# hassony2/handobjectconsist

Measured on AMD Instinct MI355X. Metric: trainmeshwarp iters/sec (render+warp, B=64, 256x256), higher is better.
Workload: dtype f32; 1 GPU; trainmeshwarp.py consist step, per-GPU B=64, 256x256, hand 778v/1552f + object 1002v/2000f (7104 faces after fill-back), ResNet-18 fp32 (MIOpen convolutions, channels-last, + fused HIP BatchNorm/ReLU/residual/max-pool kernels), Adam; global_batch=64, image_size=256, parallelism=dp1

## Files before the change

handobjectconsist_amd/_lib.py:

```python
import ctypes
import os

import torch

_HERE = os.path.dirname(os.path.abspath(__file__))
LIB_PATH = os.environ.get("HOC_LIB_PATH") or os.path.join(_HERE, "libmeshraster_hip.so")
ABI_VERSION = 9
FLAG_REFERENCE_ALGO = 1
FLAG_SPARSE_TILES = 2
FLAG_OUTPUT_ZEROED = 4
FLAG_TILE_PER_WORKGROUP = 8
FLAG_TILE_LIST_CLEARED = 16
FLAG_FORCE_PARTS = 1 << 24
FLAG_ONE_WORKGROUP_PER_IMAGE = 32 << 24
FLAG_PARTS_IN_ONE_LAUNCH = 64 << 24
FLAG_PLAIN_DIVISIONS = 4096 << 8
FLAG_FORCE_GATHER = 32 << 8
FLAG_COUNT_PIXEL_MAP_TERMS = 1024 << 8
CRITERION_L1 = 0
CRITERION_L2 = 1
DTYPE_F32, DTYPE_BF16, DTYPE_U8 = 0, 1, 2
DTYPE_CODES = {torch.float32: DTYPE_F32, torch.bfloat16: DTYPE_BF16, torch.uint8: DTYPE_U8}
IMAGE_DTYPES = (torch.float32, torch.bfloat16)
MASK_DTYPES = (torch.float32, torch.uint8)
# ... 74 lines not shown
    "mr_pair_step_field_offsets": (_I, [_P, _I]),
    "mr_pair_step_sizes": (_I, [_P, _P, _P, _P]),
    "mr_pair_step_forward": (_I, [_P, _P]),
    "mr_pair_step_backward": (_I, [_P, _P]),
    "mr_frames_to_batch_workspace_bytes": (_L, [_I, _I, _I]),
    "mr_frames_to_batch": (_I, [_P] * 3 + [_F] * 6 + [_P, _L, _P, _P] + [_I] * 6 + [_P]),
    "mr_frames_to_batch_typed": (_I, [_P] * 3 + [_F] * 6 + [_P, _L, _P, _P] + [_I] * 6 + [_P, _I, _I]),
    "mr_frames_color_augment_workspace_bytes": (_L, [_I, _I, _I]),
    "mr_frames_color_augment": (_I, [_P] * 7 + [_L, _I, _I, _I, _P]),
    "mr_jpeg_info": (_I, [_P, _L, _P]),
    "mr_jpeg_packed_bytes": (_L, [_I] * 5),
    "mr_jpeg_entropy_decode": (_I, [_P, _L, _P, _L]),
    "mr_jpeg_reconstruct_workspace_bytes": (_L, [_I] * 6),
    "mr_jpeg_reconstruct": (_I, [_P] + [_I] * 6 + [_P, _P, _L, _P]),
    "mr_png_packed_bytes": (_L, [_I] * 3),
    "mr_png_unfilter_workspace_bytes": (_L, [_I] * 4),
    "mr_png_unfilter": (_I, [_P] + [_I] * 4 + [_P, _P, _P]),
    "mr_bn_act_forward": (_I, [_P] * 6 + [_F, _I, _I, _I, _P, _I, _I, _I, _P]),
    "mr_bn_act_backward_workspace_bytes": (_L, [_I, _I]),
    "mr_bn_act_backward": (_I, [_P] * 8 + [_F, _I, _I, _I] + [_P] * 5 + [_L, _I, _I, _I, _P]),
    "mr_bn_add_bn_act_forward": (_I, [_P] * 6 + [_F] + [_P] * 4 + [_F, _I, _P, _I, _I, _I, _P]),
    "mr_bn_add_bn_act_backward_workspace_bytes": (_L, [_I, _I]),
    "mr_bn_add_bn_act_backward": (_I, [_P] * 8 + [_F] + [_P] * 4 + [_F, _I] + [_P] * 7 + [_L, _I, _I, _I, _P]),
    "mr_stem_pool_forward": (_I, [_P] * 5 + [_F, _I, _I, _P, _P, _I, _I, _I, _I, _P]),
    "mr_stem_pool_records_bytes": (_L, [_I, _I, _I, _I]),
    "mr_stem_pool_backward_workspace_bytes": (_L, [_I, _I, _I, _I]),
    "mr_stem_pool_backward": (_I, [_P] * 8 + [_F, _I, _I] + [_P] * 4 + [_L, _I, _I, _I, _I, _P]),
    "mr_stem_pool_param_grads": (_I, [_P] * 7 + [_F, _I] + [_P] * 3 + [_L, _I, _I, _I, _I, _P]),
    "mr_stem_conv_wrw_tiling": (_I, [_P] * 3),
    "mr_stem_conv_wrw_workspace_bytes": (_L, [_I, _I, _I, _I]),
    "mr_stem_conv_wrw": (_I, [_P] * 7 + [_F, _P, _P, _I, _P, _L] + [_I] * 8 + [_P]),
}

_lib = None


def load():
    global _lib
    if _lib is not None:
        return _lib
    if not os.path.exists(LIB_PATH):
        raise RuntimeError(
            f"{LIB_PATH} is missing: the HIP extension has not been built. Run "
            "`python -c 'import __graft_entry__ as g; g.build()'` (or `python handobjectconsist_amd/build.py`). "
            "There is no CPU / PyTorch fallback for the render + warp path."
        )
# ... 92 lines not shown
```

handobjectconsist_amd/csrc/frozen_bn.hip:

```cpp
#include "bn_device.hpp"

namespace mr {

struct BnParams {
    const void* x;
    const void* residual;
    BnAffine bn;
    int relu;
    int N, C, HW, split;
    void* y;
    const void* grad_y;
    const void* grad_y2;
    void* grad_x;
    void* grad_residual;
    float* partial;
};

template <bool BACKWARD>
__device__ __forceinline__ void bn_act_element(float x, bool has_res, float res, float grad, bool relu, float mean, float a,
                                               float b, float& out, float& gres, float& sum_g, float& sum_gd) {
    const float d = x - mean;
    float z = d * a + b;
    if (has_res) z = z + res;
    if (!BACKWARD) {
// ... 56 lines not shown
constexpr int BN_NHWC_BLOCKS = 2048;

template <typename T, bool BACKWARD>
__global__ __launch_bounds__(256) void bn_act_nhwc_kernel(BnParams p) {
    const NhwcLane l = nhwc_lane(p.bn, p.C);
    const int64_t pixels = (int64_t)p.N * p.HW;
    const bool relu = p.relu != 0, has_res = p.residual != nullptr;
    float s[2][4] = {};
    for (int64_t px = l.first(); px < pixels; px += l.stride()) {
        const int64_t o = px * p.C + l.c0;
        float xv[4], rv[4] = {}, gv[4] = {}, out[4], gres[4];
        load4<T>(p.x, o, xv);
        if (has_res) load4<T>(p.residual, o, rv);
        if (BACKWARD) load4_grad<T>(p.grad_y, p.grad_y2, o, gv);
#pragma unroll
        for (int i = 0; i < 4; i++)
            bn_act_element<BACKWARD>(xv[i], has_res, rv[i], gv[i], relu, l.mean[i], l.a[i], l.b[i], out[i], gres[i], s[0][i], s[1][i]);
        store4<T>(BACKWARD ? p.grad_x : p.y, o, out);
        if (BACKWARD && p.grad_residual) store4<T>(p.grad_residual, o, gres);
    }
    if (BACKWARD && p.partial) nhwc_block_sums<2>(l, s, p.partial, p.C);
}

struct BnAddParams {
    const void* x;
    const void* xd;
    BnAffine bn, bn_d;
    int N, C, HW;
    void* y;
    const void* grad_y;
    const void* grad_y2;
    void* grad_x;
    void* grad_xd;
    float* partial;
};

template <typename T, bool BACKWARD>
__global__ __launch_bounds__(256) void bn_add_bn_act_nhwc_kernel(BnAddParams p) {
    const NhwcLane l = nhwc_lane(p.bn, p.C), ld = nhwc_lane(p.bn_d, p.C);
    const int64_t pixels = (int64_t)p.N * p.HW;
    float s[3][4] = {};
    for (int64_t px = l.first(); px < pixels; px += l.stride()) {
        const int64_t o = px * p.C + l.c0;
        float xv[4], dv[4], gv[4], out[4], outd[4];
        load4<T>(p.x, o, xv);
        load4<T>(p.xd, o, dv);
// ... 99 lines not shown
    if (channels == 0) return MR_OK;
    if (!weight || !bias || !running_mean || !running_var) return MR_ERR_BADARG;
    const bool want_params = grad_weight || grad_bias;
    if (batch_size == 0 || plane == 0) return zero_param_grads({grad_weight, grad_bias}, channels, (hipStream_t)stream);
    if (!grad_y || !x || !grad_x) return MR_ERR_BADARG;
    if (grad_residual && !residual) return MR_ERR_BADARG;
    if (want_params && (!workspace || workspace_bytes < mr_bn_act_backward_workspace_bytes(batch_size, channels)))
        return MR_ERR_BADARG;
    BnParams p = bn_fill(x, residual, weight, bias, running_mean, running_var, eps, relu, batch_size, channels, plane);
    p.grad_y = grad_y; p.grad_y2 = grad_y2; p.grad_x = grad_x; p.grad_residual = grad_residual;
    p.partial = want_params ? static_cast<float*>(workspace) : nullptr;
    if (!bn_sizes_ok(p)) return MR_ERR_BADARG;
    const bool all_aligned = aligned4(x, act_dtype) && aligned4(grad_y, act_dtype) && aligned4(grad_y2, act_dtype) &&
                             aligned4(grad_x, act_dtype) && aligned4(residual, act_dtype) && aligned4(grad_residual, act_dtype);
    if (channels_last && !all_aligned) return MR_ERR_BADARG;
    const int64_t slots = bn_act_slots(batch_size, channels, channels_last, (int64_t)batch_size * plane);
    bn_launch<true>(p, act_dtype, channels_last, plane % 4 == 0 && all_aligned, (int)slots, (hipStream_t)stream);
    MR_CHECK_LAUNCH();
    if (!want_params) return MR_OK;
    return launch_bn_finish<2>(p.partial, slots, channels, BnFinishOut{running_var, eps, grad_weight, grad_bias}, (hipStream_t)stream);
}

namespace mr {
static BnAddParams bn_add_fill(const void* x, const void* xd, const BnAffine& bn, const BnAffine& bn_d, int N, int C, int plane) {
    BnAddParams p{};
    p.x = x; p.xd = xd; p.bn = bn; p.bn_d = bn_d; p.N = N; p.C = C; p.HW = plane;
    return p;
}
template <bool BACKWARD>
static void bn_add_launch(const BnAddParams& p, int act_dtype, int blocks, hipStream_t s) {
    dispatch_act(act_dtype, [&](auto tag) {
        using T = typename decltype(tag)::type;
        hipLaunchKernelGGL((bn_add_bn_act_nhwc_kernel<T, BACKWARD>), dim3((unsigned)blocks), dim3(256), 0, s, p);
    });
}
}

extern "C" int mr_bn_add_bn_act_forward(const void* x, const void* xd, const float* weight, const float* bias,
                                        const float* running_mean, const float* running_var, float eps,
                                        const float* weight_d, const float* bias_d, const float* running_mean_d,
                                        const float* running_var_d, float eps_d, int act_dtype, void* y, int batch_size,
                                        int channels, int plane, mr_stream_t stream) {
    using namespace mr;
    if (batch_size < 0 || channels < 0 || plane < 0 || (act_dtype != 0 && act_dtype != 1)) return MR_ERR_BADARG;
    if (channels > 0 && !nhwc_channels_ok(channels)) return MR_ERR_BADARG;
    if (batch_size == 0 || channels == 0 || plane == 0) return MR_OK;
// ... 53 lines not shown
```

handobjectconsist_amd/csrc/mano_lbs.hip:

```cpp
#include "mr_common.hpp"

namespace mr {

constexpr int MN_V = 778, MN_J = 16, MN_NV3 = MN_V * 3, MN_KP = 146;
constexpr int MN_TIPS = 5, MN_JT = MN_J + MN_TIPS;
constexpr int MN_SPLITK = 32;

typedef float f32x16 __attribute__((ext_vector_type(16)));

struct ManoConst {
    const float* comps;
    const float* mean;
    const float* js;
    const float* jt;
    const float* blend;
    const float* templ;
    const float* weights;
    const int* parents;
    const int* tips;
    const int* reorder;
    int ncomps, center;
};

struct ManoFull {
    const float* trans;
    int ntrans;
    float* tflag;
    float out_scale;
    const float* post_trans;
    const float* post_rot;
    const float* post_trans2;
};
constexpr int MN_POSE_PCA = 0, MN_POSE_AXISANG = 1;

__device__ __forceinline__ void rigid_mul(const float* A, const float* B, float* C) {
#pragma unroll
    for (int r = 0; r < 3; r++) {
#pragma unroll
        for (int c = 0; c < 4; c++) {
            float v = fmaf(A[4 * r + 2], B[8 + c], fmaf(A[4 * r + 1], B[4 + c], A[4 * r] * B[c]));
            if (c == 3) v += A[4 * r + 3];
            C[4 * r + c] = v;
        }
    }
}

template <int FORM, bool FULL>
__global__ void __launch_bounds__(64) mano_pre_kernel(ManoConst mc, ManoFull mf, const float* __restrict__ pose,
                                                      const float* __restrict__ betas, float* __restrict__ coeff,
                                                      float* __restrict__ G, float* __restrict__ G2,
                                                      float* __restrict__ rots, float* __restrict__ joints,
                                                      float* __restrict__ full_pose_out, float* __restrict__ jtr_out,
                                                      int B) {
    __shared__ float s_pose[48], s_R[MN_J * 9], s_J[48], s_G[MN_J * 12];
    const int b = blockIdx.x, lane = threadIdx.x;
    const int np = FORM == MN_POSE_AXISANG ? 48 : 3 + mc.ncomps;
    if (lane < 3) s_pose[lane] = pose[b * np + lane];
    if (lane < 45) {
        if constexpr (FORM == MN_POSE_AXISANG) {
            s_pose[3 + lane] = mc.mean[lane] + pose[b * np + 3 + lane];
        } else {
            float acc = 0.0f;
            for (int c = 0; c < mc.ncomps; c++) acc = fmaf(pose[b * np + 3 + c], mc.comps[c * 45 + lane], acc);
            s_pose[3 + lane] = mc.mean[lane] + acc;
        }
    }
    if constexpr (FULL) {
        unsigned bits = 0u;
        for (int i = lane; i < mf.ntrans; i += 64) bits |= __float_as_uint(mf.trans[i]) & 0x7fffffffu;
        const bool in_force = __ballot(bits != 0u) != 0ull;
        if (lane == 0) mf.tflag[b] = in_force ? 1.0f : 0.0f;
    }
    if (lane < 48) {
        float acc = 0.0f;
#pragma unroll
        for (int k = 0; k < 10; k++) acc = fmaf(betas[b * 10 + k], mc.js[lane * 10 + k], acc);
        s_J[lane] = acc + mc.jt[lane];
    }
    __syncthreads();
    if (lane < 48) {
        full_pose_out[b * 48 + lane] = s_pose[lane];
        joints[b * 48 + lane] = s_J[lane];
    }
    if (lane < MN_J) {
        float R[9];
        rodrigues(&s_pose[3 * lane], R, nullptr);
#pragma unroll
        for (int k = 0; k < 9; k++) {
            s_R[lane * 9 + k] = R[k];
            rots[(b * MN_J + lane) * 9 + k] = R[k];
            if (lane > 0) coeff[b * MN_KP + 10 + (lane - 1) * 9 + k] = R[k] - ((k == 0 || k == 4 || k == 8) ? 1.0f : 0.0f);
        }
    }
    if (lane < 10) coeff[b * MN_KP + lane] = betas[b * 10 + lane];
    if (lane == 10) coeff[b * MN_KP + MN_KP - 1] = 0.0f;
    __syncthreads();
    if (lane == 0) {
        for (int j = 0; j < MN_J; j++) {
            const int pa = mc.parents[j];
            float rel[12];
#pragma unroll
            for (int r = 0; r < 3; r++) {
#pragma unroll
                for (int c = 0; c < 3; c++) rel[4 * r + c] = s_R[j * 9 + 3 * r + c];
                rel[4 * r + 3] = pa < 0 ? s_J[3 * j + r] : s_J[3 * j + r] - s_J[3 * pa + r];
            }
            if (pa < 0) {
#pragma unroll
                for (int k = 0; k < 12; k++) s_G[j * 12 + k] = rel[k];
            } else {
                rigid_mul(&s_G[pa * 12], rel, &s_G[j * 12]);
            }
        }
    }
    __syncthreads();
    for (int k = lane; k < MN_J * 12; k += 64) {
        const int j = k / 12, e = k % 12, r = e / 4, c = e % 4;
        float v = s_G[k];
        G[b * MN_J * 12 + k] = v;
        if (c == 3)
            v = v - fmaf(s_G[j * 12 + 4 * r + 2], s_J[3 * j + 2],
                         fmaf(s_G[j * 12 + 4 * r + 1], s_J[3 * j + 1], s_G[j * 12 + 4 * r] * s_J[3 * j]));
        G2[b * MN_J * 12 + k] = v;
    }
    if constexpr (!FULL) {
        if (lane < MN_JT * 3) {
            const int k = lane / 3, r = lane % 3, src = mc.reorder[k];
            if (src < MN_J) {
                const float ctr = mc.center >= 0 ? s_G[mc.center * 12 + 4 * r + 3] : 0.0f;
                jtr_out[(b * MN_JT + k) * 3 + r] = (s_G[src * 12 + 4 * r + 3] - ctr) * 1000.0f;
            }
        }
    }
}

__global__ void __launch_bounds__(64) mano_blend_kernel(const float* __restrict__ coeff, const float* __restrict__ blend,
                                                        const float* __restrict__ templ, float* __restrict__ v_posed,
                                                        int B) {
    const int lane = threadIdx.x;
    const int n0 = blockIdx.x * 32, m0 = blockIdx.y * 32;
    const int i = lane & 31, kh = lane >> 5;
    const int row = min(m0 + i, B - 1), col = min(n0 + i, MN_NV3 - 1);
    f32x16 acc = {0, 0, 0, 0, 0, 0, 0, 0, 0, 0, 0, 0, 0, 0, 0, 0};
#pragma unroll 4
    for (int k = 0; k < MN_KP; k += 2) {
        const float a = coeff[row * MN_KP + k + kh];
        const float bb = blend[(k + kh) * MN_NV3 + col];
        acc = __builtin_amdgcn_mfma_f32_32x32x2f32(a, bb, acc, 0, 0, 0);
    }
    const int n = n0 + i;
// ... 221 lines not shown
        acc = __builtin_amdgcn_mfma_f32_32x32x2f32(a, bb, acc, 0, 0, 0);
    }
    const int n = n0 + i;
#pragma unroll
    for (int r = 0; r < 16; r++) {
        const int m = m0 + (r & 3) + 8 * (r >> 2) + 4 * kh;
        if (m < Mpad && n < 160) partial[((int64_t)s * Mpad + m) * 160 + n] = acc[r];
    }
}

template <int FORM, bool FULL>
__global__ void __launch_bounds__(64) mano_pre_bwd_kernel(ManoConst mc, ManoFull mf, float* __restrict__ grad_trans,
                                                          const float* __restrict__ full_pose,
                                                          const float* __restrict__ rots,
                                                          const float* __restrict__ joints, const float* __restrict__ G,
                                                          const float* __restrict__ part,
                                                          const float* __restrict__ partial,
                                                          const float* __restrict__ grad_jtr,
                                                          float* __restrict__ grad_pose, float* __restrict__ grad_betas,
                                                          int B, int Mpad) {
    __shared__ double s_gG2[MN_J * 12], s_gc[3], s_gcoef[MN_KP], s_gG[MN_J * 12], s_gRd[MN_J * 9], s_gJ[48], s_gt[MN_J][3];
    __shared__ float s_gR[MN_J * 9], s_gp[48];
    __shared__ float s_G[MN_J * 12], s_R[MN_J * 9], s_J[48];
    const int b = blockIdx.x, lane = threadIdx.x;
    const int np = FORM == MN_POSE_AXISANG ? 48 : 3 + mc.ncomps;
    for (int k = lane; k < MN_J * 12; k += 64) {
        double acc = 0.0;
        for (int c = 0; c < MN_CHUNKS; c++) acc += (double)part[((int64_t)b * MN_CHUNKS + c) * MN_PART + k];
        s_gG2[k] = acc;
        s_G[k] = G[b * MN_J * 12 + k];
    }
    if (lane < 3) {
        double acc = 0.0;
        for (int c = 0; c < MN_CHUNKS; c++) acc += (double)part[((int64_t)b * MN_CHUNKS + c) * MN_PART + MN_J * 12 + lane];
        s_gc[lane] = acc;
    }
    for (int k = lane; k < MN_KP; k += 64) {
        double acc = 0.0;
        for (int s = 0; s < MN_SPLITK; s++) acc += (double)partial[((int64_t)s * Mpad + b) * 160 + k];
        s_gcoef[k] = acc;
    }
    for (int k = lane; k < MN_J * 9; k += 64) s_R[k] = rots[b * MN_J * 9 + k];
    if (lane < 48) { s_J[lane] = joints[b * 48 + lane]; s_gJ[lane] = 0.0; }
    __syncthreads();
    if (lane == 0) {
        double (*gt)[3] = s_gt;
        for (int j = 0; j < MN_J; j++) gt[j][0] = gt[j][1] = gt[j][2] = 0.0;
        double gc[3] = {s_gc[0], s_gc[1], s_gc[2]};
        if (grad_jtr)
            for (int k = 0; k < MN_JT; k++) {
                const int src = mc.reorder[k];
                for (int r = 0; r < 3; r++) {
                    const double g = (double)grad_jtr[(b * MN_JT + k) * 3 + r] * 1000.0;
                    if (src < MN_J) { gt[src][r] += g; gc[r] -= g; }
                }
            }
        if constexpr (FULL) {
            const bool in_force = mf.tflag[b] != 0.0f;
            if (grad_trans)
                for (int r = 0; r < 3; r++) grad_trans[b * 3 + r] = in_force ? (float)(0.0 - gc[r]) : 0.0f;
            if (mc.center >= 0 && mc.center < MN_J && !in_force)
                for (int r = 0; r < 3; r++) gt[mc.center][r] += gc[r];
        } else {
            if (mc.center >= 0)
                for (int r = 0; r < 3; r++) gt[mc.center][r] += gc[r];
        }
        for (int j = 0; j < MN_J; j++) {
            for (int r = 0; r < 3; r++) {
                const double gt2 = s_gG2[j * 12 + 4 * r + 3];
                for (int c = 0; c < 3; c++) {
                    s_gG[j * 12 + 4 * r + c] = s_gG2[j * 12 + 4 * r + c] - gt2 * (double)s_J[3 * j + c];
                    s_gJ[3 * j + c] -= (double)s_G[j * 12 + 4 * r + c] * gt2;
                }
                s_gG[j * 12 + 4 * r + 3] = gt2 + gt[j][r];
            }
        }
        for (int j = MN_J - 1; j >= 0; j--) {
            const int pa = mc.parents[j];
            if (pa < 0) {
                for (int r = 0; r < 3; r++) {
                    for (int c = 0; c < 3; c++) s_gRd[j * 9 + 3 * r + c] = s_gG[j * 12 + 4 * r + c];
                    s_gJ[3 * j + r] += s_gG[j * 12 + 4 * r + 3];
                }
                continue;
            }
            double rel[12];
            for (int r = 0; r < 3; r++) {
                for (int c = 0; c < 3; c++) rel[4 * r + c] = (double)s_R[j * 9 + 3 * r + c];
                rel[4 * r + 3] = (double)s_J[3 * j + r] - (double)s_J[3 * pa + r];
            }
            for (int r = 0; r < 3; r++)
                for (int c = 0; c < 4; c++) {
                    double acc = 0.0;
                    for (int k = 0; k < 3; k++) acc += (double)s_G[pa * 12 + 4 * k + r] * s_gG[j * 12 + 4 * k + c];
                    if (c < 3) s_gRd[j * 9 + 3 * r + c] = acc;
                    else { s_gJ[3 * j + r] += acc; s_gJ[3 * pa + r] -= acc; }
                }
            for (int r = 0; r < 3; r++) {
                for (int c = 0; c < 3; c++) {
                    double acc = 0.0;
                    for (int k = 0; k < 4; k++) acc += s_gG[j * 12 + 4 * r + k] * rel[4 * c + k];
                    s_gG[pa * 12 + 4 * r + c] += acc;
                }
                s_gG[pa * 12 + 4 * r + 3] += s_gG[j * 12 + 4 * r + 3];
            }
        }
    }
    __syncthreads();
    for (int k = lane; k < MN_J * 9; k += 64) s_gR[k] = (float)(k >= 9 ? s_gRd[k] + s_gcoef[10 + (k - 9)] : s_gRd[k]);
    __syncthreads();
    if (lane < MN_J) {
        float gr[3];
        rodrigues_bwd(&full_pose[b * 48 + 3 * lane], &s_gR[lane * 9], gr);
#pragma unroll
        for (int k = 0; k < 3; k++) s_gp[3 * lane + k] = gr[k];
    }
    __syncthreads();
    if (lane < 3) grad_pose[b * np + lane] = s_gp[lane];
    if constexpr (FORM == MN_POSE_AXISANG) {
        if (lane < 45) grad_pose[b * np + 3 + lane] = s_gp[3 + lane];
    } else if (lane < mc.ncomps) {
        float acc = 0.0f;
        for (int l = 0; l < 45; l++) acc = fmaf(mc.comps[lane * 45 + l], s_gp[3 + l], acc);
        grad_pose[b * np + 3 + lane] = acc;
    }
    if (lane < 10) {
        double acc = s_gcoef[lane];
        for (int l = 0; l < 48; l++) acc += (double)mc.js[l * 10 + lane] * s_gJ[l];
        grad_betas[b * 10 + lane] = (float)acc;
    }
}

}

using namespace mr;

static ManoConst mano_const(const float* comps, const float* mean, const float* js, const float* jt, const float* blend,
                            const float* templ, const float* weights, const int32_t* parents, const int32_t* tips,
                            const int32_t* reorder, int ncomps, int center) {
    return ManoConst{comps, mean, js, jt, blend, templ, weights, (const int*)parents, (const int*)tips, (const int*)reorder,
                     ncomps, center};
}

struct ManoWork {
    float *coeff, *G, *G2, *rots, *joints, *full_pose, *v_posed, *grad_vp, *part, *partial;
    float* tflag;
    int Mpad;
    int64_t floats, full_floats;
};
static ManoWork mano_work(float* w, int64_t B) {
// ... 167 lines not shown
```

handobjectconsist_amd/models/synthnet.py:

```python
import os

import numpy as np
import torch
import torch.nn.functional as F
from torch import nn

from handobjectconsist_amd import _lib
from handobjectconsist_amd.nn import frozen_bn
from handobjectconsist_amd.utils import project as camproject
from handobjectconsist_amd.utils import synth


USE_HIP_BN = os.environ.get("HOC_HIP_BN", "1") == "1"


USE_CHANNELS_LAST = os.environ.get("HOC_CHANNELS_LAST", "1") == "1"


USE_STEM_WRW = True


def _fused_bn(bn, x):
    if not (USE_HIP_BN and not bn.training and x.is_cuda):
        return False
    out_dtype = torch.get_autocast_dtype("cuda") if torch.is_autocast_enabled("cuda") else x.dtype
    return out_dtype in (torch.float32, torch.bfloat16)


class BasicBlock(nn.Module):
    expansion = 1

    def __init__(self, inplanes, planes, stride=1, downsample=None):
        super().__init__()
        self.conv1 = nn.Conv2d(inplanes, planes, 3, stride, 1, bias=False)
        self.bn1 = nn.BatchNorm2d(planes)
        self.relu = nn.ReLU(inplace=True)
        self.conv2 = nn.Conv2d(planes, planes, 3, 1, 1, bias=False)
        self.bn2 = nn.BatchNorm2d(planes)
        self.downsample = downsample

    def forward_fused(self, x, x_identity, dup=False):
        if self.downsample is not None:
            xd = self.downsample[0](x_identity)
            out = frozen_bn.bn_act(self.conv1(x), self.bn1)
            return frozen_bn.bn_add_bn_act(self.conv2(out), self.bn2, xd, self.downsample[1], dup=dup)
        out = frozen_bn.bn_act(self.conv1(x), self.bn1)
        return frozen_bn.bn_act(self.conv2(out), self.bn2, residual=x_identity, dup=dup)

    def forward(self, x):
        if _fused_bn(self.bn1, x):
            return self.forward_fused(x, x)
        residual = x if self.downsample is None else self.downsample(x)
        out = self.relu(self.bn1(self.conv1(x)))
        out = self.bn2(self.conv2(out))
        return self.relu(out + residual)


class ResNet18Features(nn.Module):

    def __init__(self):
        super().__init__()
        self.inplanes = 64
        self.conv1 = nn.Conv2d(3, 64, kernel_size=7, stride=2, padding=3, bias=False)
        self.bn1 = nn.BatchNorm2d(64)
        self.relu = nn.ReLU(inplace=True)
        self.maxpool = nn.MaxPool2d(kernel_size=3, stride=2, padding=1)
        self.layer1 = self._make_layer(64, 2)
        self.layer2 = self._make_layer(128, 2, stride=2)
        self.layer3 = self._make_layer(256, 2, stride=2)
        self.layer4 = self._make_layer(512, 2, stride=2)
# ... 4 lines not shown
    def _make_layer(self, planes, blocks, stride=1):
        downsample = None
        if stride != 1 or self.inplanes != planes:
            downsample = nn.Sequential(nn.Conv2d(self.inplanes, planes, 1, stride, bias=False),
                                       nn.BatchNorm2d(planes))
        layers = [BasicBlock(self.inplanes, planes, stride, downsample)]
        self.inplanes = planes
        layers += [BasicBlock(planes, planes) for _ in range(1, blocks)]
        return nn.Sequential(*layers)

    def forward(self, x):
        if USE_CHANNELS_LAST and x.is_cuda:
            if not self.conv1.weight.is_contiguous(memory_format=torch.channels_last):
                self.to(memory_format=torch.channels_last)
            x = x.contiguous(memory_format=torch.channels_last)
        if _fused_bn(self.bn1, x):
            blocks = [b for layer in (self.layer1, self.layer2, self.layer3, self.layer4) for b in layer]
            if USE_STEM_WRW and frozen_bn.conv_stem_applies(x, self.conv1, self.bn1):
                pair = frozen_bn.conv_stem_pool(x, self.conv1, self.bn1, dup=True)
            else:
                pair = frozen_bn.stem_pool(self.conv1(x), self.bn1, dup=True)
            for block in blocks[:-1]:
                pair = block.forward_fused(pair[0], pair[1], dup=True)
            x = blocks[-1].forward_fused(pair[0], pair[1])
        else:
            x = self.maxpool(self.relu(self.bn1(self.conv1(x))))
            x = self.layer4(self.layer3(self.layer2(self.layer1(x))))
        return x.mean(3).mean(2)


class AbsoluteBranch(nn.Module):

    def __init__(self, base_neurons=(512, 256), out_dim=3):
        super().__init__()
        layers = []
        for i, o in zip(base_neurons[:-1], base_neurons[1:]):
            layers += [nn.Linear(i, o), nn.ReLU()]
        self.decoder = nn.Sequential(*layers)
        self.final_layer = nn.Linear(base_neurons[-1], out_dim)

    def forward(self, inp):
        return self.final_layer(self.decoder(inp))


def batch_rodrigues(rvec):
    angle = torch.norm(rvec + 1e-8, p=2, dim=1, keepdim=True)
    axis = rvec / angle
    half = angle * 0.5
    q = torch.cat([torch.cos(half), torch.sin(half) * axis], 1)
    q = q / q.norm(p=2, dim=1, keepdim=True)
# ... 439 lines not shown
```

handobjectconsist_amd/nn/frozen_bn.py:

```python
import torch
import torch.nn.functional as F

from handobjectconsist_amd import _lib


_ACT_DTYPES = {torch.float32: 0, torch.bfloat16: 1}


def _nhwc_channels_ok(C):
    return 4 <= C <= 1024 and 1024 % C == 0


def _layout(x):
    if (x.dim() == 4 and _nhwc_channels_ok(x.shape[1]) and not x.is_contiguous()
            and x.is_contiguous(memory_format=torch.channels_last)):
        return x, 1
    return x.contiguous(), 0


def _aligned(t, cl):
    if t is not None and cl and t.data_ptr() % (4 * t.element_size()):
        return t.clone(memory_format=torch.preserve_format)
    return t

# ... 51 lines not shown
        xc, rc, w, b, m, v = ctx.saved_tensors
        eps, relu, N, C, plane, cl = ctx.cfg
        need_x, need_r, need_w, need_b = ctx.needs_input_grad[:4]
        g, g2 = _incoming(grad_y, grad_y2, xc.dtype, cl)
        if g is None:
            return (None,) * 9
        dev = xc.device
        grad_x = torch.empty_like(xc)
        grad_r = torch.empty_like(xc) if (rc is not None and need_r) else None
        grad_w = torch.empty_like(w) if need_w else None
        grad_b = torch.empty_like(b) if need_b else None
        work, wbytes = _workspace("mr_bn_act_backward_workspace_bytes", (N, C), dev, need_w or need_b)
        _lib.call("mr_bn_act_backward", _lib.ptr(g), _lib.ptr(g2), _lib.ptr(xc), _lib.ptr(rc), _lib.ptr(w), _lib.ptr(b), _lib.ptr(m),
                  _lib.ptr(v), eps, int(relu), _ACT_DTYPES[xc.dtype], cl, _lib.ptr(grad_x), _lib.ptr(grad_r), _lib.ptr(grad_w),
                  _lib.ptr(grad_b),
                  _lib.ptr(work), wbytes, N, C, plane, _lib.stream_ptr(dev))
        return (grad_x if need_x else None), grad_r, grad_w, grad_b, None, None, None, None, None


def bn_act(x, bn, residual=None, relu=True, dup=False):
    if bn.training or not bn.track_running_stats:
        raise RuntimeError("bn_act needs frozen BatchNorm statistics (module.eval())")
    return _BnActFunction.apply(x, residual, bn.weight, bn.bias, bn.running_mean, bn.running_var, bn.eps, relu, dup)


class _BnAddBnActFunction(torch.autograd.Function):

    @staticmethod
    def forward(ctx, x, xd, weight, bias, running_mean, running_var, eps, weight_d, bias_d, running_mean_d,
                running_var_d, eps_d, dup):
        ctx.set_materialize_grads(False)
        _lib.check_cuda(x, xd, weight, bias, running_mean, running_var, weight_d, bias_d, running_mean_d, running_var_d)
        xc, xdc = _aligned(x, 1), _aligned(xd, 1)
        N, C = xc.shape[:2]
        plane = xc[0, 0].numel() if N and C else 0
        chan = _channel_arrays(C, weight, bias, running_mean, running_var, weight_d, bias_d, running_mean_d, running_var_d)
        y = torch.empty_like(xc)
        _lib.call("mr_bn_add_bn_act_forward", _lib.ptr(xc), _lib.ptr(xdc), *[_lib.ptr(t) for t in chan[:4]], float(eps),
                  *[_lib.ptr(t) for t in chan[4:]], float(eps_d), _ACT_DTYPES[xc.dtype], _lib.ptr(y), N, C, plane,
                  _lib.stream_ptr(xc.device))
        ctx.save_for_backward(xc, xdc, *chan)
        ctx.cfg = (float(eps), float(eps_d), N, C, plane)
        return (y, y.view_as(y)) if dup else y

    @staticmethod
    def backward(ctx, grad_y, grad_y2=None):
# ... 152 lines not shown
```

include/meshraster_hip.h:

```cpp
#ifndef MESHRASTER_HIP_H
#define MESHRASTER_HIP_H

#include <stdint.h>

#ifdef __cplusplus
extern "C" {
#endif

#define MR_OK 0
#define MR_ERR_BADARG (-1)
#define MR_ERR_NOTIMPL (-2)

#define MR_FLAG_REFERENCE_ALGO 1
#define MR_FLAG_SPARSE_TILES 2
#define MR_FLAG_OUTPUT_ZEROED 4
#define MR_FLAG_TILE_PER_WORKGROUP 8
#define MR_FLAG_TILE_LIST_CLEARED 16
#define MR_FLAG_FORCE_PARTS (1 << 24)
#define MR_FLAG_ONE_WORKGROUP_PER_IMAGE (32 << 24)
#define MR_FLAG_PARTS_IN_ONE_LAUNCH (64 << 24)
#define MR_FLAG_PLAIN_DIVISIONS (4096 << 8)
#define MR_FLAG_FORCE_GATHER (32 << 8)
#define MR_FLAG_COUNT_PIXEL_MAP_TERMS (1024 << 8)

// ... 481 lines not shown
MR_API int mr_bn_act_backward(const void* grad_y, const void* grad_y2, const void* x, const void* residual,
                              const float* weight, const float* bias, const float* running_mean,
                              const float* running_var, float eps, int relu, int act_dtype,
                              int channels_last, void* grad_x, void* grad_residual, float* grad_weight,
                              float* grad_bias,
                              void* workspace, int64_t workspace_bytes, int batch_size, int channels,
                              int plane, mr_stream_t stream);

MR_API int mr_bn_add_bn_act_forward(const void* x, const void* xd, const float* weight, const float* bias,
                                    const float* running_mean, const float* running_var, float eps,
                                    const float* weight_d, const float* bias_d, const float* running_mean_d,
                                    const float* running_var_d, float eps_d, int act_dtype, void* y,
                                    int batch_size, int channels, int plane, mr_stream_t stream);
MR_API int64_t mr_bn_add_bn_act_backward_workspace_bytes(int batch_size, int channels);
MR_API int mr_bn_add_bn_act_backward(const void* grad_y, const void* grad_y2, const void* x, const void* xd,
                                     const float* weight, const float* bias, const float* running_mean,
                                     const float* running_var, float eps, const float* weight_d,
                                     const float* bias_d, const float* running_mean_d, const float* running_var_d,
                                     float eps_d, int act_dtype, void* grad_x, void* grad_xd, float* grad_weight,
                                     float* grad_bias, float* grad_weight_d, float* grad_bias_d, void* workspace,
                                     int64_t workspace_bytes, int batch_size, int channels, int plane,
                                     mr_stream_t stream);

MR_API int mr_stem_pool_forward(const void* x, const float* weight, const float* bias,
                                const float* running_mean, const float* running_var, float eps,
                                int act_dtype, int channels_last, void* y, unsigned char* argmax,
                                int batch_size, int channels, int height, int width, mr_stream_t stream);
MR_API int64_t mr_stem_pool_records_bytes(int batch_size, int channels, int height, int width);
MR_API int64_t mr_stem_pool_backward_workspace_bytes(int batch_size, int channels, int height, int width);
MR_API int mr_stem_pool_backward(const void* grad_y, const void* grad_y2, const void* x,
                                 const unsigned char* argmax,
                                 const float* weight, const float* bias, const float* running_mean,
                                 const float* running_var, float eps, int act_dtype, int channels_last,
                                 void* grad_x, float* grad_weight, float* grad_bias, void* workspace,
                                 int64_t workspace_bytes, int batch_size, int channels, int height,
                                 int width, mr_stream_t stream);

MR_API int mr_stem_pool_param_grads(const void* grad_y, const void* grad_y2, const unsigned char* records,
                                    const float* weight, const float* bias, const float* running_mean,
                                    const float* running_var, float eps, int act_dtype, float* grad_weight,
                                    float* grad_bias, void* workspace, int64_t workspace_bytes, int batch_size,
                                    int channels, int height, int width, mr_stream_t stream);

MR_API int mr_stem_conv_wrw_tiling(int* tile_height, int* tile_width, int* workgroups);
MR_API int64_t mr_stem_conv_wrw_workspace_bytes(int batch_size, int channels, int in_height, int in_width);
MR_API int mr_stem_conv_wrw(const float* grad_y, const float* grad_y2, const unsigned char* records,
// ... 11 lines not shown
```

Before: 38.58 iters/s (one optimiser step = 1 data batch + 1 consist batch of B per GPU; roofline.stock_trunk_it_s = the same step with the trunk's BatchNorm/ReLU/max-pool on the stock nn modules).

## Fuse final BN/ReLU/residual with global average pool and parallelise MANO kinematic chain

Adds a fused kernel that applies the last block's frozen BatchNorm, residual add and ReLU and directly reduces to pooled features. Its backward broadcasts the pooled gradient inside the BN backward, which removes the full-size activation write and the separate mean reductions at the trunk exit. It also rewrites the MANO forward and backward kinematic-chain passes from a single serial lane to level-by-level parallel work over chain depth. That adds extra shared memory and syncthreads in exchange. The layer4 output is tiny (8x8), so the gain from the fusion is likely small.

```diff
diff --git a/handobjectconsist_amd/_lib.py b/handobjectconsist_amd/_lib.py
--- a/handobjectconsist_amd/_lib.py
+++ b/handobjectconsist_amd/_lib.py
@@ -120,6 +120,8 @@
     "mr_bn_add_bn_act_forward": (_I, [_P] * 6 + [_F] + [_P] * 4 + [_F, _I, _P, _I, _I, _I, _P]),
     "mr_bn_add_bn_act_backward_workspace_bytes": (_L, [_I, _I]),
     "mr_bn_add_bn_act_backward": (_I, [_P] * 8 + [_F] + [_P] * 4 + [_F, _I] + [_P] * 7 + [_L, _I, _I, _I, _P]),
+    "mr_bn_act_pool_forward": (_I, [_P] * 6 + [_F, _P, _I, _I, _I, _I, _P]),
+    "mr_bn_act_pool_backward": (_I, [_P] * 7 + [_F] + [_P] * 5 + [_L, _I, _I, _I, _I, _P]),
     "mr_stem_pool_forward": (_I, [_P] * 5 + [_F, _I, _I, _P, _P, _I, _I, _I, _I, _P]),
     "mr_stem_pool_records_bytes": (_L, [_I, _I, _I, _I]),
     "mr_stem_pool_backward_workspace_bytes": (_L, [_I, _I, _I, _I]),
diff --git a/handobjectconsist_amd/csrc/frozen_bn.hip b/handobjectconsist_amd/csrc/frozen_bn.hip
--- a/handobjectconsist_amd/csrc/frozen_bn.hip
+++ b/handobjectconsist_amd/csrc/frozen_bn.hip
@@ -102,6 +102,89 @@
     if (BACKWARD && p.partial) nhwc_block_sums<2>(l, s, p.partial, p.C);
 }
 
+struct BnPoolParams {
+    const float* x;
+    const float* residual;
+    BnAffine bn;
+    int N, C, H, W;
+    float inv_h, inv_w;
+    float* features;
+    const float* grad_features;
+    float* grad_x;
+    float* grad_residual;
+    float* partial;
+};
+
+template <int S>
+__device__ __forceinline__ void pool_tree(float (&t)[S][4]) {
+#pragma unroll
+    for (int step = 1; step < S; step *= 2)
+#pragma unroll
+        for (int j = 0; j < S; j += 2 * step)
+#pragma unroll
+            for (int i = 0; i < 4; i++) t[j][i] = t[j][i] + t[j + step][i];
+}
+
+template <int S>
+__global__ __launch_bounds__(256) void bn_act_pool_forward_kernel(BnPoolParams p) {
+    const int groups = p.C >> 2;
+    const int64_t t = (int64_t)blockIdx.x * 256 + threadIdx.x;
+    if (t >= (int64_t)p.N * groups) return;
+    const int n = (int)(t / groups), c0 = 4 * (int)(t % groups);
+    float mean[4], a[4], b[4];
+#pragma unroll
+    for (int i = 0; i < 4; i++) channel_consts(p.bn, c0 + i, mean[i], a[i], b[i]);
+    const bool has_res = p.residual != nullptr;
+    float rows[S][4];
+#pragma unroll
+    for (int h = 0; h < S; h++) {
+        float row[S][4];
+#pragma unroll
+        for (int w = 0; w < S; w++) {
+            const int64_t o = (((int64_t)n * S + h) * S + w) * p.C + c0;
+            float xv[4], rv[4] = {};
+            load4<float>(p.x, o, xv);
+            if (has_res) load4<float>(p.residual, o, rv);
+#pragma unroll
+            for (int i = 0; i < 4; i++) {
+                float gres, s0 = 0.0f, s1 = 0.0f;
+                bn_act_element<false>(xv[i], has_res, rv[i], 0.0f, true, mean[i], a[i], b[i], row[w][i], gres, s0, s1);
+            }
+        }
+        pool_tree<S>(row);
+#pragma unroll
+        for (int i = 0; i < 4; i++) rows[h][i] = row[0][i] * p.inv_w;
+    }
+    pool_tree<S>(rows);
+    float f[4];
+#pragma unroll
+    for (int i = 0; i < 4; i++) f[i] = rows[0][i] * p.inv_h;
+    store4<float>(p.features, (int64_t)n * p.C + c0, f);
+}
+
+__global__ __launch_bounds__(256) void bn_act_pool_backward_kernel(BnPoolParams p) {
+    const NhwcLane l = nhwc_lane(p.bn, p.C);
+    const int HW = p.H * p.W;
+    const int64_t pixels = (int64_t)p.N * HW;
+    const bool has_res = p.residual != nullptr;
+    float s[2][4] = {};
+    for (int64_t px = l.first(); px < pixels; px += l.stride()) {
+        const int64_t o = px * p.C + l.c0;
+        float xv[4], rv[4] = {}, gv[4], out[4], gres[4];
+        load4<float>(p.x, o, xv);
+        if (has_res) load4<float>(p.residual, o, rv);
+        load4<float>(p.grad_features, (px / HW) * p.C + l.c0, gv);
+#pragma unroll
+        for (int i = 0; i < 4; i++) {
+            const float g = (gv[i] * p.inv_h) * p.inv_w;
+            bn_act_element<true>(xv[i], has_res, rv[i], g, true, l.mean[i], l.a[i], l.b[i], out[i], gres[i], s[0][i], s[1][i]);
+        }
+        store4<float>(p.grad_x, o, out);
+        if (p.grad_residual) store4<float>(p.grad_residual, o, gres);
+    }
+    if (p.partial) nhwc_block_sums<2>(l, s, p.partial, p.C);
+}
+
 struct BnAddParams {
     const void* x;
     const void* xd;
@@ -247,6 +330,77 @@
 }
 
 namespace mr {
+static int bn_pool_check(int N, int C, int H, int W, std::initializer_list<const void*> ptrs) {
+    if (N < 0 || C < 0 || H < 0 || W < 0) return MR_ERR_BADARG;
+    if (C > 0 && !nhwc_channels_ok(C)) return MR_ERR_BADARG;
+    if ((int64_t)H * W > 0x7fffffff || (int64_t)N * C > 0x7fffffff) return MR_ERR_BADARG;
+    for (const void* q : ptrs)
+        if (!aligned4(q, 0)) return MR_ERR_BADARG;
+    return MR_OK;
+}
+static BnPoolParams bn_pool_fill(const void* x, const void* residual, const float* weight, const float* bias, const float* mean,
+                                 const float* var, float eps, int N, int C, int H, int W) {
+    BnPoolParams p{};
+    p.x = static_cast<const float*>(x); p.residual = static_cast<const float*>(residual);
+    p.bn = BnAffine{weight, bias, mean, var, eps};
+    p.N = N; p.C = C; p.H = H; p.W = W;
+    p.inv_h = 1.0f / (float)H; p.inv_w = 1.0f / (float)W;
+    return p;
+}
+}
+
+extern "C" int mr_bn_act_pool_forward(const void* x, const void* residual, const float* weight, const float* bias,
+                                      const float* running_mean, const float* running_var, float eps, float* features,
+                                      int batch_size, int channels, int height, int width, mr_stream_t stream) {
+    using namespace mr;
+    const int rc = bn_pool_check(batch_size, channels, height, width, {x, residual, features});
+    if (rc != MR_OK) return rc;
+    if (batch_size == 0 || channels == 0) return MR_OK;
+    if (height == 0 || width == 0) return MR_ERR_BADARG;
+    if (!x || !weight || !bias || !running_mean || !running_var || !features) return MR_ERR_BADARG;
+    if (height != width || (height != 1 && height != 2 && height != 4 && height != 8)) return MR_ERR_NOTIMPL;
+    BnPoolParams p = bn_pool_fill(x, residual, weight, bias, running_mean, running_var, eps, batch_size, channels, height, width);
+    p.features = features;
+    const dim3 grid((unsigned)(((int64_t)batch_size * (channels / 4) + 255) / 256));
+    switch (height) {
+        case 1: hipLaunchKernelGGL(bn_act_pool_forward_kernel<1>, grid, dim3(256), 0, (hipStream_t)stream, p); break;
+        case 2: hipLaunchKernelGGL(bn_act_pool_forward_kernel<2>, grid, dim3(256), 0, (hipStream_t)stream, p); break;
+        case 4: hipLaunchKernelGGL(bn_act_pool_forward_kernel<4>, grid, dim3(256), 0, (hipStream_t)stream, p); break;
+        default: hipLaunchKernelGGL(bn_act_pool_forward_kernel<8>, grid, dim3(256), 0, (hipStream_t)stream, p); break;
+    }
+    MR_CHECK_LAUNCH();
+    return MR_OK;
+}
+
+extern "C" int mr_bn_act_pool_backward(const float* grad_features, const void* x, const void* residual, const float* weight,
+                                       const float* bias, const float* running_mean, const float* running_var, float eps,
+                                       void* grad_x, void* grad_residual, float* grad_weight, float* grad_bias,
+                                       void* workspace, int64_t workspace_bytes, int batch_size, int channels, int height,
+                                       int width, mr_stream_t stream) {
+    using namespace mr;
+    const int rc = bn_pool_check(batch_size, channels, height, width, {grad_features, x, residual, grad_x, grad_residual});
+    if (rc != MR_OK) return rc;
+    if (channels == 0) return MR_OK;
+    if (!weight || !bias || !running_mean || !running_var) return MR_ERR_BADARG;
+    const bool want_params = grad_weight || grad_bias;
+    if (batch_size == 0) return zero_param_grads({grad_weight, grad_bias}, channels, (hipStream_t)stream);
+    if (height == 0 || width == 0) return MR_ERR_BADARG;
+    if (!grad_features || !x || !grad_x) return MR_ERR_BADARG;
+    if (grad_residual && !residual) return MR_ERR_BADARG;
+    if (want_params && (!workspace || workspace_bytes < mr_bn_act_backward_workspace_bytes(batch_size, channels)))
+        return MR_ERR_BADARG;
+    BnPoolParams p = bn_pool_fill(x, residual, weight, bias, running_mean, running_var, eps, batch_size, channels, height, width);
+    p.grad_features = grad_features;
+    p.grad_x = static_cast<float*>(grad_x); p.grad_residual = static_cast<float*>(grad_residual);
+    p.partial = want_params ? static_cast<float*>(workspace) : nullptr;
+    const int64_t slots = bn_act_slots(batch_size, channels, 1, (int64_t)batch_size * height * width);
+    hipLaunchKernelGGL(bn_act_pool_backward_kernel, dim3((unsigned)slots), dim3(256), 0, (hipStream_t)stream, p);
+    MR_CHECK_LAUNCH();
+    if (!want_params) return MR_OK;
+    return launch_bn_finish<2>(p.partial, slots, channels, BnFinishOut{running_var, eps, grad_weight, grad_bias}, (hipStream_t)stream);
+}
+
+namespace mr {
 static BnAddParams bn_add_fill(const void* x, const void* xd, const BnAffine& bn, const BnAffine& bn_d, int N, int C, int plane) {
     BnAddParams p{};
     p.x = x; p.xd = xd; p.bn = bn; p.bn_d = bn_d; p.N = N; p.C = C; p.HW = plane;
diff --git a/handobjectconsist_amd/csrc/mano_lbs.hip b/handobjectconsist_amd/csrc/mano_lbs.hip
--- a/handobjectconsist_amd/csrc/mano_lbs.hip
+++ b/handobjectconsist_amd/csrc/mano_lbs.hip
@@ -45,6 +45,20 @@
     }
 }
 
+__device__ __forceinline__ int chain_depths(int parent, int* s_par, int* s_depth, int lane) {
+    if (lane < MN_J) s_par[lane] = parent;
+    __syncthreads();
+    if (lane < MN_J) {
+        int d = 0;
+        for (int p = s_par[lane]; p >= 0 && p < MN_J && d < MN_J; p = s_par[p]) d++;
+        s_depth[lane] = d;
+    }
+    __syncthreads();
+    int maxd = 0;
+    for (int j = 0; j < MN_J; j++) maxd = max(maxd, s_depth[j]);
+    return maxd;
+}
+
 template <int FORM, bool FULL>
 __global__ void __launch_bounds__(64) mano_pre_kernel(ManoConst mc, ManoFull mf, const float* __restrict__ pose,
                                                       const float* __restrict__ betas, float* __restrict__ coeff,
@@ -53,8 +67,11 @@
                                                       float* __restrict__ full_pose_out, float* __restrict__ jtr_out,
                                                       int B) {
     __shared__ float s_pose[48], s_R[MN_J * 9], s_J[48], s_G[MN_J * 12];
+    __shared__ int s_par[MN_J], s_depth[MN_J];
     const int b = blockIdx.x, lane = threadIdx.x;
     const int np = FORM == MN_POSE_AXISANG ? 48 : 3 + mc.ncomps;
+    const int parent = lane < MN_J ? mc.parents[lane] : -1;
+    const int src = !FULL && lane < MN_JT * 3 ? mc.reorder[lane / 3] : MN_J;
     if (lane < 3) s_pose[lane] = pose[b * np + lane];
     if (lane < 45) {
         if constexpr (FORM == MN_POSE_AXISANG) {
@@ -94,26 +111,26 @@
     }
     if (lane < 10) coeff[b * MN_KP + lane] = betas[b * 10 + lane];
     if (lane == 10) coeff[b * MN_KP + MN_KP - 1] = 0.0f;
-    __syncthreads();
-    if (lane == 0) {
-        for (int j = 0; j < MN_J; j++) {
-            const int pa = mc.parents[j];
-            float rel[12];
-#pragma unroll
-            for (int r = 0; r < 3; r++) {
-#pragma unroll
-                for (int c = 0; c < 3; c++) rel[4 * r + c] = s_R[j * 9 + 3 * r + c];
-                rel[4 * r + 3] = pa < 0 ? s_J[3 * j + r] : s_J[3 * j + r] - s_J[3 * pa + r];
+    const int maxd = chain_depths(parent, s_par, s_depth, lane);
+    for (int d = 0; d <= maxd; d++) {
+        for (int k = lane; k < MN_J * 12; k += 64) {
+            const int j = k / 12, r = (k % 12) / 4, c = k % 4;
+            if (s_depth[j] != d) continue;
+            const int pa = s_par[j];
+            float rel[3];
+#pragma unroll
+            for (int i = 0; i < 3; i++)
+                rel[i] = c < 3 ? s_R[j * 9 + 3 * i + c] : (pa < 0 ? s_J[3 * j + i] : s_J[3 * j + i] - s_J[3 * pa + i]);
+            float v = rel[r];
+            if (pa >= 0) {
+                const float* A = &s_G[pa * 12];
+                v = fmaf(A[4 * r + 2], rel[2], fmaf(A[4 * r + 1], rel[1], A[4 * r] * rel[0]));
+                if (c == 3) v += A[4 * r + 3];
             }
-            if (pa < 0) {
-#pragma unroll
-                for (int k = 0; k < 12; k++) s_G[j * 12 + k] = rel[k];
-            } else {
-                rigid_mul(&s_G[pa * 12], rel, &s_G[j * 12]);
-            }
-        }
-    }
-    __syncthreads();
+            s_G[k] = v;
+        }
+        __syncthreads();
+    }
     for (int k = lane; k < MN_J * 12; k += 64) {
         const int j = k / 12, e = k % 12, r = e / 4, c = e % 4;
         float v = s_G[k];
@@ -125,7 +142,7 @@
     }
     if constexpr (!FULL) {
         if (lane < MN_JT * 3) {
-            const int k = lane / 3, r = lane % 3, src = mc.reorder[k];
+            const int k = lane / 3, r = lane % 3;
             if (src < MN_J) {
                 const float ctr = mc.center >= 0 ? s_G[mc.center * 12 + 4 * r + 3] : 0.0f;
                 jtr_out[(b * MN_JT + k) * 3 + r] = (s_G[src * 12 + 4 * r + 3] - ctr) * 1000.0f;
@@ -393,96 +410,122 @@
     __shared__ double s_gG2[MN_J * 12], s_gc[3], s_gcoef[MN_KP], s_gG[MN_J * 12], s_gRd[MN_J * 9], s_gJ[48], s_gt[MN_J][3];
     __shared__ float s_gR[MN_J * 9], s_gp[48];
     __shared__ float s_G[MN_J * 12], s_R[MN_J * 9], s_J[48];
+    __shared__ double s_gjt[MN_JT * 3], s_up[MN_J * 12], s_gJrel[48];
+    __shared__ int s_src[MN_JT], s_par[MN_J], s_depth[MN_J];
     const int b = blockIdx.x, lane = threadIdx.x;
     const int np = FORM == MN_POSE_AXISANG ? 48 : 3 + mc.ncomps;
+    const int parent = lane < MN_J ? mc.parents[lane] : -1;
+    const int src = lane < MN_JT ? mc.reorder[lane] : 0, src3 = lane < MN_JT * 3 ? mc.reorder[lane / 3] : MN_J;
+    const float gjt = grad_jtr && lane < MN_JT * 3 ? grad_jtr[b * MN_JT * 3 + lane] : 0.0f;
+    float axisang[3] = {0.0f, 0.0f, 0.0f};
+    if (lane < MN_J)
+#pragma unroll
+        for (int k = 0; k < 3; k++) axisang[k] = full_pose[b * 48 + 3 * lane + k];
     for (int k = lane; k < MN_J * 12; k += 64) {
         double acc = 0.0;
+#pragma unroll
         for (int c = 0; c < MN_CHUNKS; c++) acc += (double)part[((int64_t)b * MN_CHUNKS + c) * MN_PART + k];
         s_gG2[k] = acc;
         s_G[k] = G[b * MN_J * 12 + k];
     }
     if (lane < 3) {
         double acc = 0.0;
+#pragma unroll
         for (int c = 0; c < MN_CHUNKS; c++) acc += (double)part[((int64_t)b * MN_CHUNKS + c) * MN_PART + MN_J * 12 + lane];
         s_gc[lane] = acc;
     }
     for (int k = lane; k < MN_KP; k += 64) {
         double acc = 0.0;
+#pragma unroll
         for (int s = 0; s < MN_SPLITK; s++) acc += (double)partial[((int64_t)s * Mpad + b) * 160 + k];
         s_gcoef[k] = acc;
     }
     for (int k = lane; k < MN_J * 9; k += 64) s_R[k] = rots[b * MN_J * 9 + k];
-    if (lane < 48) { s_J[lane] = joints[b * 48 + lane]; s_gJ[lane] = 0.0; }
-    __syncthreads();
-    if (lane == 0) {
-        double (*gt)[3] = s_gt;
-        for (int j = 0; j < MN_J; j++) gt[j][0] = gt[j][1] = gt[j][2] = 0.0;
-        double gc[3] = {s_gc[0], s_gc[1], s_gc[2]};
-        if (grad_jtr)
-            for (int k = 0; k < MN_JT; k++) {
-                const int src = mc.reorder[k];
-                for (int r = 0; r < 3; r++) {
-                    const double g = (double)grad_jtr[(b * MN_JT + k) * 3 + r] * 1000.0;
-                    if (src < MN_J) { gt[src][r] += g; gc[r] -= g; }
+    if (lane < 48) s_J[lane] = joints[b * 48 + lane];
+    if (lane < MN_JT) s_src[lane] = src;
+    if (lane < MN_JT * 3) s_gjt[lane] = src3 < MN_J ? (double)gjt * 1000.0 : 0.0;
+    const int maxd = chain_depths(parent, s_par, s_depth, lane);
+    if (lane < 48) {
+        const int j = lane / 3, r = lane % 3;
+        double g = 0.0;
+        for (int k = 0; k < MN_JT; k++)
+            if (s_src[k] == j) g += s_gjt[3 * k + r];
+        s_gt[j][r] = g;
+    } else if (lane < 51) {
+        const int r = lane - 48;
+        double gc = s_gc[r];
+        for (int k = 0; k < MN_JT; k++) gc -= s_gjt[3 * k + r];
+        s_gc[r] = gc;
+    }
+    __syncthreads();
+    if (lane < 3) {
+        const int r = lane;
+        const double gc = s_gc[r];
+        if constexpr (FULL) {
+            const bool in_force = mf.tflag[b] != 0.0f;
+            if (grad_trans) grad_trans[b * 3 + r] = in_force ? (float)(0.0 - gc) : 0.0f;
+            if (mc.center >= 0 && mc.center < MN_J && !in_force) s_gt[mc.center][r] += gc;
+        } else {
+            if (mc.center >= 0) s_gt[mc.center][r] += gc;
+        }
+    }
+    __syncthreads();
+    if (lane < 48) {
+        const int j = lane / 3, r = lane % 3;
+        const double gt2 = s_gG2[j * 12 + 4 * r + 3];
+        for (int c = 0; c < 3; c++) s_gG[j * 12 + 4 * r + c] = s_gG2[j * 12 + 4 * r + c] - gt2 * (double)s_J[3 * j + c];
+        s_gG[j * 12 + 4 * r + 3] = gt2 + s_gt[j][r];
+        double gj = 0.0;
+        for (int rr = 0; rr < 3; rr++) gj -= (double)s_G[j * 12 + 4 * rr + r] * s_gG2[j * 12 + 4 * rr + 3];
+        s_gJ[lane] = gj;
+    }
+    __syncthreads();
+    for (int d = maxd; d >= 1; d--) {
+        for (int k = lane; k < MN_J * 12; k += 64) {
+            const int j = k / 12, r = (k % 12) / 4, c = k % 4;
+            if (s_depth[j] != d) continue;
+            const int pa = s_par[j];
+            double acc = 0.0;
+            for (int i = 0; i < 3; i++) acc += (double)s_G[pa * 12 + 4 * i + r] * s_gG[j * 12 + 4 * i + c];
+            if (c < 3) s_gRd[j * 9 + 3 * r + c] = acc;
+            else s_gJrel[3 * j + r] = acc;
+            double up = s_gG[j * 12 + 4 * r + 3];
+            if (c < 3) {
+                up = 0.0;
+                for (int i = 0; i < 4; i++) {
+                    const double rel = i < 3 ? (double)s_R[j * 9 + 3 * c + i] : (double)s_J[3 * j + c] - (double)s_J[3 * pa + c];
+                    up += s_gG[j * 12 + 4 * r + i] * rel;
                 }
             }
-        if constexpr (FULL) {
-            const bool in_force = mf.tflag[b] != 0.0f;
-            if (grad_trans)
-                for (int r = 0; r < 3; r++) grad_trans[b * 3 + r] = in_force ? (float)(0.0 - gc[r]) : 0.0f;
-            if (mc.center >= 0 && mc.center < MN_J && !in_force)
-                for (int r = 0; r < 3; r++) gt[mc.center][r] += gc[r];
-        } else {
-            if (mc.center >= 0)
-                for (int r = 0; r < 3; r++) gt[mc.center][r] += gc[r];
-        }
-        for (int j = 0; j < MN_J; j++) {
-            for (int r = 0; r < 3; r++) {
-                const double gt2 = s_gG2[j * 12 + 4 * r + 3];
-                for (int c = 0; c < 3; c++) {
-                    s_gG[j * 12 + 4 * r + c] = s_gG2[j * 12 + 4 * r + c] - gt2 * (double)s_J[3 * j + c];
-                    s_gJ[3 * j + c] -= (double)s_G[j * 12 + 4 * r + c] * gt2;
-                }
-                s_gG[j * 12 + 4 * r + 3] = gt2 + gt[j][r];
-            }
-        }
-        for (int j = MN_J - 1; j >= 0; j--) {
-            const int pa = mc.parents[j];
-            if (pa < 0) {
-                for (int r = 0; r < 3; r++) {
-                    for (int c = 0; c < 3; c++) s_gRd[j * 9 + 3 * r + c] = s_gG[j * 12 + 4 * r + c];
-                    s_gJ[3 * j + r] += s_gG[j * 12 + 4 * r + 3];
-                }
-                continue;
-            }
-            double rel[12];
-            for (int r = 0; r < 3; r++) {
-                for (int c = 0; c < 3; c++) rel[4 * r + c] = (double)s_R[j * 9 + 3 * r + c];
-                rel[4 * r + 3] = (double)s_J[3 * j + r] - (double)s_J[3 * pa + r];
-            }
-            for (int r = 0; r < 3; r++)
-                for (int c = 0; c < 4; c++) {
-                    double acc = 0.0;
-                    for (int k = 0; k < 3; k++) acc += (double)s_G[pa * 12 + 4 * k + r] * s_gG[j * 12 + 4 * k + c];
-                    if (c < 3) s_gRd[j * 9 + 3 * r + c] = acc;
-                    else { s_gJ[3 * j + r] += acc; s_gJ[3 * pa + r] -= acc; }
-                }
-            for (int r = 0; r < 3; r++) {
-                for (int c = 0; c < 3; c++) {
-                    double acc = 0.0;
-                    for (int k = 0; k < 4; k++) acc += s_gG[j * 12 + 4 * r + k] * rel[4 * c + k];
-                    s_gG[pa * 12 + 4 * r + c] += acc;
-                }
-                s_gG[pa * 12 + 4 * r + 3] += s_gG[j * 12 + 4 * r + 3];
-            }
-        }
+            s_up[k] = up;
+        }
+        __syncthreads();
+        for (int k = lane; k < MN_J * 12; k += 64) {
+            const int p = k / 12;
+            if (s_depth[p] != d - 1) continue;
+            double v = s_gG[k];
+            for (int j = MN_J - 1; j > p; j--)
+                if (s_par[j] == p) v += s_up[j * 12 + k % 12];
+            s_gG[k] = v;
+        }
+        __syncthreads();
+    }
+    for (int k = lane; k < MN_J * 9; k += 64)
+        if (s_par[k / 9] < 0) s_gRd[k] = s_gG[(k / 9) * 12 + 4 * ((k % 9) / 3) + k % 3];
+    if (lane < 48) {
+        const int l = lane / 3, r = lane % 3;
+        double v = s_gJ[lane];
+        for (int j = MN_J - 1; j > l; j--)
+            if (s_par[j] == l) v -= s_gJrel[3 * j + r];
+        v += s_par[l] < 0 ? s_gG[l * 12 + 4 * r + 3] : s_gJrel[lane];
+        s_gJ[lane] = v;
     }
     __syncthreads();
     for (int k = lane; k < MN_J * 9; k += 64) s_gR[k] = (float)(k >= 9 ? s_gRd[k] + s_gcoef[10 + (k - 9)] : s_gRd[k]);
     __syncthreads();
     if (lane < MN_J) {
         float gr[3];
-        rodrigues_bwd(&full_pose[b * 48 + 3 * lane], &s_gR[lane * 9], gr);
+        rodrigues_bwd(axisang, &s_gR[lane * 9], gr);
 #pragma unroll
         for (int k = 0; k < 3; k++) s_gp[3 * lane + k] = gr[k];
     }
@@ -492,11 +535,13 @@
         if (lane < 45) grad_pose[b * np + 3 + lane] = s_gp[3 + lane];
     } else if (lane < mc.ncomps) {
         float acc = 0.0f;
+#pragma unroll
         for (int l = 0; l < 45; l++) acc = fmaf(mc.comps[lane * 45 + l], s_gp[3 + l], acc);
         grad_pose[b * np + 3 + lane] = acc;
     }
     if (lane < 10) {
         double acc = s_gcoef[lane];
+#pragma unroll
         for (int l = 0; l < 48; l++) acc += (double)mc.js[l * 10 + lane] * s_gJ[l];
         grad_betas[b * 10 + lane] = (float)acc;
     }
diff --git a/handobjectconsist_amd/models/synthnet.py b/handobjectconsist_amd/models/synthnet.py
--- a/handobjectconsist_amd/models/synthnet.py
+++ b/handobjectconsist_amd/models/synthnet.py
@@ -18,6 +18,9 @@
 
 
 USE_STEM_WRW = True
+
+
+USE_POOLED_EXIT = True
 
 
 def _fused_bn(bn, x):
@@ -39,13 +42,17 @@
         self.bn2 = nn.BatchNorm2d(planes)
         self.downsample = downsample
 
-    def forward_fused(self, x, x_identity, dup=False):
+    def forward_fused(self, x, x_identity, dup=False, pool=False):
         if self.downsample is not None:
             xd = self.downsample[0](x_identity)
             out = frozen_bn.bn_act(self.conv1(x), self.bn1)
-            return frozen_bn.bn_add_bn_act(self.conv2(out), self.bn2, xd, self.downsample[1], dup=dup)
+            out = frozen_bn.bn_add_bn_act(self.conv2(out), self.bn2, xd, self.downsample[1], dup=dup)
+            return out.mean(3).mean(2) if pool else out
         out = frozen_bn.bn_act(self.conv1(x), self.bn1)
-        return frozen_bn.bn_act(self.conv2(out), self.bn2, residual=x_identity, dup=dup)
+        if pool and USE_POOLED_EXIT:
+            return frozen_bn.bn_act_pool(self.conv2(out), self.bn2, residual=x_identity)
+        out = frozen_bn.bn_act(self.conv2(out), self.bn2, residual=x_identity, dup=dup)
+        return out.mean(3).mean(2) if pool else out
 
     def forward(self, x):
         if _fused_bn(self.bn1, x):
@@ -96,10 +103,9 @@
                 pair = frozen_bn.stem_pool(self.conv1(x), self.bn1, dup=True)
             for block in blocks[:-1]:
                 pair = block.forward_fused(pair[0], pair[1], dup=True)
-            x = blocks[-1].forward_fused(pair[0], pair[1])
-        else:
-            x = self.maxpool(self.relu(self.bn1(self.conv1(x))))
-            x = self.layer4(self.layer3(self.layer2(self.layer1(x))))
+            return blocks[-1].forward_fused(pair[0], pair[1], pool=True)
+        x = self.maxpool(self.relu(self.bn1(self.conv1(x))))
+        x = self.layer4(self.layer3(self.layer2(self.layer1(x))))
         return x.mean(3).mean(2)
 
 
diff --git a/handobjectconsist_amd/nn/frozen_bn.py b/handobjectconsist_amd/nn/frozen_bn.py
--- a/handobjectconsist_amd/nn/frozen_bn.py
+++ b/handobjectconsist_amd/nn/frozen_bn.py
@@ -97,6 +97,53 @@
     if bn.training or not bn.track_running_stats:
         raise RuntimeError("bn_act needs frozen BatchNorm statistics (module.eval())")
     return _BnActFunction.apply(x, residual, bn.weight, bn.bias, bn.running_mean, bn.running_var, bn.eps, relu, dup)
+
+
+POOLED_EXIT_SIZES = frozenset({(1, 1), (2, 2), (4, 4), (8, 8)})
+
+
+class _BnActPoolFunction(torch.autograd.Function):
+
+    @staticmethod
+    def forward(ctx, x, residual, weight, bias, running_mean, running_var, eps):
+        _lib.check_cuda(x, residual, weight, bias, running_mean, running_var)
+        xc = _aligned(x, 1)
+        rc = _aligned(residual.contiguous(memory_format=torch.channels_last), 1) if residual is not None else None
+        N, C, H, W = xc.shape
+        w, b, m, v = _channel_arrays(C, weight, bias, running_mean, running_var)
+        features = torch.empty((N, C), dtype=torch.float32, device=xc.device)
+        _lib.call("mr_bn_act_pool_forward", _lib.ptr(xc), _lib.ptr(rc), _lib.ptr(w), _lib.ptr(b), _lib.ptr(m), _lib.ptr(v),
+                  float(eps), _lib.ptr(features), N, C, H, W, _lib.stream_ptr(xc.device))
+        ctx.save_for_backward(xc, rc, w, b, m, v)
+        ctx.cfg = (float(eps), N, C, H, W)
+        return features
+
+    @staticmethod
+    def backward(ctx, grad_features):
+        xc, rc, w, b, m, v = ctx.saved_tensors
+        eps, N, C, H, W = ctx.cfg
+        need_x, need_r, need_w, need_b = ctx.needs_input_grad[:4]
+        g = grad_features.float().contiguous()
+        dev = xc.device
+        grad_x = torch.empty_like(xc)
+        grad_r = torch.empty_like(xc) if (rc is not None and need_r) else None
+        grad_w = torch.empty_like(w) if need_w else None
+        grad_b = torch.empty_like(b) if need_b else None
+        work, wbytes = _workspace("mr_bn_act_backward_workspace_bytes", (N, C), dev, need_w or need_b)
+        _lib.call("mr_bn_act_pool_backward", _lib.ptr(g), _lib.ptr(xc), _lib.ptr(rc), _lib.ptr(w), _lib.ptr(b), _lib.ptr(m),
+                  _lib.ptr(v), eps, _lib.ptr(grad_x), _lib.ptr(grad_r), _lib.ptr(grad_w), _lib.ptr(grad_b), _lib.ptr(work),
+                  wbytes, N, C, H, W, _lib.stream_ptr(dev))
+        return (grad_x if need_x else None), grad_r, grad_w, grad_b, None, None, None
+
+
+def bn_act_pool(x, bn, residual=None):
+    if bn.training or not bn.track_running_stats:
+        raise RuntimeError("bn_act_pool needs frozen BatchNorm statistics (module.eval())")
+    if (x.dim() == 4 and x.is_cuda and x.dtype == torch.float32 and x.numel() > 0 and _layout(x)[1]
+            and tuple(x.shape[2:]) in POOLED_EXIT_SIZES
+            and (residual is None or (residual.shape == x.shape and residual.dtype == x.dtype))):
+        return _BnActPoolFunction.apply(x, residual, bn.weight, bn.bias, bn.running_mean, bn.running_var, bn.eps)
+    return bn_act(x, bn, residual=residual).mean(3).mean(2)
 
 
 class _BnAddBnActFunction(torch.autograd.Function):
diff --git a/include/meshraster_hip.h b/include/meshraster_hip.h
--- a/include/meshraster_hip.h
+++ b/include/meshraster_hip.h
@@ -527,6 +527,15 @@
                                      int64_t workspace_bytes, int batch_size, int channels, int plane,
                                      mr_stream_t stream);
 
+MR_API int mr_bn_act_pool_forward(const void* x, const void* residual, const float* weight, const float* bias,
+                                  const float* running_mean, const float* running_var, float eps, float* features,
+                                  int batch_size, int channels, int height, int width, mr_stream_t stream);
+MR_API int mr_bn_act_pool_backward(const float* grad_features, const void* x, const void* residual,
+                                   const float* weight, const float* bias, const float* running_mean,
+                                   const float* running_var, float eps, void* grad_x, void* grad_residual,
+                                   float* grad_weight, float* grad_bias, void* workspace, int64_t workspace_bytes,
+                                   int batch_size, int channels, int height, int width, mr_stream_t stream);
+
 MR_API int mr_stem_pool_forward(const void* x, const float* weight, const float* bias,
                                 const float* running_mean, const float* running_var, float eps,
                                 int act_dtype, int channels_last, void* y, unsigned char* argmax,
```

New measurement: 38.94 iters/s (one optimiser step = 1 data batch + 1 consist batch of B per GPU; roofline.stock_trunk_it_s = the same step with the trunk's BatchNorm/ReLU/max-pool on the stock nn modules), median of 6. No clear change (+0.9%).
